# RuanJohn/Mava

Measured on AMD Instinct MI355X. Metric: env-steps/sec (whole node), ff_mappo RWARE tiny-4ag, higher is better.
Workload: dtype f32 via 2 x f16 split operands on the MFMA (3 products, f32 accumulate); 1 GPU; ff_mappo RWARE tiny-4ag-shaped synthetic obs, 4096 envs/GPU (update_batch_size=1 x num_envs=4096), rollout_length=128, ppo_epochs=4, num_minibatches=2, agents=4, obs=70/264, actions=5, one step = one PPO update = 524288 env-steps per GPU; parallelism=dp1

## Files before the change

### include/mava_hip.h

```cpp
#ifndef MAVA_HIP_H
#define MAVA_HIP_H

#include <stddef.h>
#include <stdint.h>

#ifdef __cplusplus
extern "C" {
#endif

typedef struct ihipStream_t* mava_stream_t;

const char* mava_last_error(void);
int mava_abi_version(void);

typedef struct mava_ctx mava_ctx;
enum {
  MAVA_CTX_MATMUL_MODE = 0,
  MAVA_CTX_CRITIC_AGGREGATION = 1,
  MAVA_CTX_GAE_VARIANT = 2,
  MAVA_CTX_POLICY_VARIANT = 3,
  MAVA_CTX_H2_LAUNCHES = 4,
  MAVA_CTX_TRAIN_VARIANT = 5,
  MAVA_CTX_W8_LAUNCHES = 6,
  MAVA_CTX_W1_SPLIT_FRESH = 7,
  MAVA_CTX_EXACT_TILES = 8
};
int mava_ctx_create(mava_ctx** out);
int mava_ctx_destroy(mava_ctx* ctx);
int mava_ctx_set(mava_ctx* ctx, int key, long value);
int mava_ctx_get(const mava_ctx* ctx, int key, long* value);

int mava_gae_f32(const mava_ctx* ctx, const float* reward, const float* value, const uint8_t* done,
                 const float* last_val, const uint8_t* last_done, int T, int N, float gamma,
                 float lambda, float* adv, float* tgt, mava_stream_t s);

int mava_permutation_i32(long n, uint64_t seed, uint64_t counter, int32_t* out, mava_stream_t s);

int mava_clip_adam(float* p, const float* g, float* m, float* v, int32_t* count,
                   const int* seg_off, const float* seg_lr, int n_seg, float grad_scale,
                   float max_norm, int decay, int steps_per_update, int num_updates, float b1,
// ... 363 lines not shown
```

### mava_amd/_lib.py

```python
from __future__ import annotations

import ctypes as C
import os
from typing import Optional

import torch

_HERE = os.path.dirname(os.path.abspath(__file__))
LIB_PATH = os.environ.get("MAVA_LIB_PATH") or os.path.join(_HERE, "libmavahip.so")

_lib: Optional[C.CDLL] = None


class MavaHipError(RuntimeError):
    pass


vp = C.c_void_p
i32 = C.c_int
u32 = C.c_uint32
u64 = C.c_uint64
f32 = C.c_float
lng = C.c_long

# ... 111 lines not shown
            )
        _lib = C.CDLL(LIB_PATH)
        _lib.mava_last_error.restype = C.c_char_p
        _lib.mava_last_error.argtypes = []
        for name, args in _SIGNATURES.items():
            fn = getattr(_lib, name)
            fn.argtypes = args
            fn.restype = _RESTYPES.get(name, C.c_int)
    return _lib


class Ctx:

    MATMUL_MODE, CRITIC_AGGREGATION, GAE_VARIANT, POLICY_VARIANT, H2_LAUNCHES, TRAIN_VARIANT, W8_LAUNCHES, W1_SPLIT_FRESH = 0, 1, 2, 3, 4, 5, 6, 7
    EXACT_TILES = 8

    def __init__(self, matmul_mode: str = "f32", critic_aggregation: bool = True):
        if matmul_mode not in ("f32", "f16x2"):
            raise ValueError(f"matmul_mode must be 'f16x2' or 'f32', got {matmul_mode!r}")
        h = C.c_void_p()
        check(lib().mava_ctx_create(C.byref(h)), "mava_ctx_create")
        self.handle: Optional[int] = h.value
        self.set(self.MATMUL_MODE, 1 if matmul_mode == "f16x2" else 0)
        self.set(self.CRITIC_AGGREGATION, int(bool(critic_aggregation)))

    def set(self, key: int, value: int) -> None:
        check(lib().mava_ctx_set(self.handle, key, int(value)), "mava_ctx_set")

    def get(self, key: int) -> int:
        out = C.c_long()
# ... 59 lines not shown
```

### mava_amd/csrc/api.cpp

```cpp
#include <stdarg.h>
#include <stdio.h>
#include <string.h>

#include "common.h"
#include "ctx.h"

static thread_local char g_err[512] = "";

void mava_set_error(const char* fmt, ...) {
  va_list ap;
  va_start(ap, fmt);
  vsnprintf(g_err, sizeof(g_err), fmt, ap);
  va_end(ap);
}

extern "C" const char* mava_last_error(void) { return g_err; }

extern "C" int mava_abi_version(void) { return 3; }

enum { CTX_MATMUL_MODE = 0, CTX_CRITIC_AGGREGATION = 1, CTX_GAE_VARIANT = 2, CTX_POLICY_VARIANT = 3, CTX_H2_LAUNCHES = 4, CTX_TRAIN_VARIANT = 5, CTX_W8_LAUNCHES = 6, CTX_W1_SPLIT_FRESH = 7, CTX_EXACT_TILES = 8 };

extern "C" int mava_ctx_create(mava_ctx** out) {
  MAVA_ARG_CHECK(out != nullptr, 0, "mava_ctx_create: null output pointer");
  mava_ctx* c = new mava_ctx();
  c->matmul_mode = 0;
  c->critic_aggregation = 1;
  c->gae_variant = 0;
  c->policy_variant = 0;
  c->h2_launches = 0;
  c->train_variant = 0;
  c->w8_launches = 0;
  c->w1_split[0] = c->w1_split[1] = nullptr;
  for (int i = 0; i < 2; ++i) {
    c->w1_fresh[i] = 0;
    c->w1_key_params[i] = nullptr;
    c->w1_key_din[i] = c->w1_key_steps[i] = 0;
  }
  c->exact_tiles = nullptr;
  *out = c;
  return MAVA_OK;
}

extern "C" int mava_ctx_destroy(mava_ctx* c) {
  if (c == nullptr) return MAVA_OK;
  for (int i = 0; i < 2; ++i)
    if (c->w1_split[i] != nullptr) (void)hipFree(c->w1_split[i]);
  if (c->exact_tiles != nullptr) (void)hipFree(c->exact_tiles);
  delete c;
  return MAVA_OK;
}

extern "C" int mava_ctx_set(mava_ctx* c, int key, long value) {
  MAVA_ARG_CHECK(c != nullptr, 0, "mava_ctx_set: null context");
  switch (key) {
    case CTX_MATMUL_MODE:
      MAVA_ARG_CHECK(value == 0 || value == 1, 1, "mava_ctx_set: matmul mode %ld (0 = exact f32, 1 = f16x2)", value);
      c->matmul_mode = (int)value;
      c->w1_fresh[0] = c->w1_fresh[1] = 0;
      return MAVA_OK;
    case CTX_CRITIC_AGGREGATION: c->critic_aggregation = value ? 1 : 0; return MAVA_OK;
    case CTX_GAE_VARIANT: c->gae_variant = (int)value; return MAVA_OK;
    case CTX_POLICY_VARIANT: c->policy_variant = (int)value; return MAVA_OK;
    case CTX_H2_LAUNCHES: c->h2_launches = value; return MAVA_OK;
    case CTX_TRAIN_VARIANT: c->train_variant = (int)value; return MAVA_OK;
    case CTX_W8_LAUNCHES: c->w8_launches = value; return MAVA_OK;
    case CTX_W1_SPLIT_FRESH:
      MAVA_ARG_CHECK(value == 0, 1, "mava_ctx_set: MAVA_CTX_W1_SPLIT_FRESH can only be cleared (0) by the caller");
      c->w1_fresh[0] = c->w1_fresh[1] = 0;
      return MAVA_OK;
    case CTX_EXACT_TILES:
      MAVA_ARG_CHECK(value == 0, 1, "mava_ctx_set: MAVA_CTX_EXACT_TILES can only be reset (0) by the caller");
      if (c->exact_tiles != nullptr) {
        MAVA_HIP_CHECK(hipDeviceSynchronize());
        MAVA_HIP_CHECK(hipMemset(c->exact_tiles, 0, sizeof(unsigned long long)));
      }
      return MAVA_OK;
    default: mava_set_error("mava_ctx_set: unknown key %d", key); return MAVA_EARG(2);
  }
}

extern "C" int mava_ctx_get(const mava_ctx* c, int key, long* value) {
  MAVA_ARG_CHECK(c != nullptr && value != nullptr, 0, "mava_ctx_get: null argument");
  switch (key) {
    case CTX_MATMUL_MODE: *value = c->matmul_mode; return MAVA_OK;
    case CTX_CRITIC_AGGREGATION: *value = c->critic_aggregation; return MAVA_OK;
    case CTX_GAE_VARIANT: *value = c->gae_variant; return MAVA_OK;
    case CTX_POLICY_VARIANT: *value = c->policy_variant; return MAVA_OK;
    case CTX_H2_LAUNCHES: *value = c->h2_launches; return MAVA_OK;
    case CTX_TRAIN_VARIANT: *value = c->train_variant; return MAVA_OK;
    case CTX_W8_LAUNCHES: *value = c->w8_launches; return MAVA_OK;
    case CTX_W1_SPLIT_FRESH: *value = c->w1_fresh[1]; return MAVA_OK;
    case CTX_EXACT_TILES: {
      unsigned long long n = 0;
      if (c->exact_tiles != nullptr) {
        MAVA_HIP_CHECK(hipDeviceSynchronize());
        MAVA_HIP_CHECK(hipMemcpy(&n, c->exact_tiles, sizeof(n), hipMemcpyDeviceToHost));
      }
      *value = (long)n;
      return MAVA_OK;
    }
    default: mava_set_error("mava_ctx_get: unknown key %d", key); return MAVA_EARG(2);
  }
}
```

### mava_amd/csrc/ctx.h

```cpp
#pragma once
#include "common.h"

struct mava_ctx {
  int matmul_mode;
  int critic_aggregation;
  int gae_variant;
  int policy_variant;
  int train_variant;
  long h2_launches;
  long w8_launches;
  void* w1_split[2];
  int w1_fresh[2];
  const float* w1_key_params[2];
  int w1_key_din[2];
  int w1_key_steps[2];
  unsigned long long* exact_tiles;
};

static inline int mava_ctx_matmul_mode(const mava_ctx* c) { return c ? c->matmul_mode : 0; }
static inline int mava_ctx_critic_aggregation(const mava_ctx* c) { return c ? c->critic_aggregation : 1; }
static inline int mava_ctx_gae_variant(const mava_ctx* c) { return c ? c->gae_variant : 0; }
static inline int mava_ctx_policy_variant(const mava_ctx* c) { return c ? c->policy_variant : 0; }
```

### mava_amd/csrc/ppo_train_h2.hip

```cpp
#include "h2_core.h"
#include "ppo_train_task.h"
#include "ctx.h"

#include <type_traits>

#ifndef MAVA_GW_DEPTH
#define MAVA_GW_DEPTH 0
#endif
#define GW_DEPTH MAVA_GW_DEPTH
#ifndef MAVA_GW_DEPTH_WIDE
#define MAVA_GW_DEPTH_WIDE 0
#endif

namespace {

using namespace h2;

constexpr int STATS_BLOCKS = 128;

#ifdef MAVA_STAMPS
#define STAMP_DECL unsigned long long st_prev = __builtin_readcyclecounter(), st_acc[16] = {0, 0, 0, 0, 0, 0, 0, 0, 0, 0, 0, 0, 0, 0, 0, 0};
#define STAMP(i)                                                    \
  do {                                                              \
    __builtin_amdgcn_sched_barrier(0);                              \
// ... 1010 lines not shown
    if (tk.action_f != nullptr) return 1;
    if (tk.no <= 8) return dispatch_s1<8, true>(ctx, tk, n_slab, s);
#ifndef MAVA_FAST_BUILD
    if (tk.no <= 16) return dispatch_s1<16, true>(ctx, tk, n_slab, s);
    return dispatch_s1<32, true>(ctx, tk, n_slab, s);
#else
    return 1;
#endif
  }
  return dispatch_s1<1, false>(ctx, tk, n_slab, s);
}

int mava_train_h2_launch(mava_ctx* ctx, const TrainTask& tk_in, int n_slab, bool actor, hipStream_t s) {
  TrainTask tk = tk_in;
  tk.force_xlo = (ctx->train_variant & 2) != 0;
  if ((ctx->train_variant & 1) == 0) {
    const int rc8 = mava_train_w8_launch(tk, n_slab, actor, s);
    if (rc8 <= 0) {
      if (rc8 == 0) { ++ctx->h2_launches; ++ctx->w8_launches; }
      return rc8;
    }
  }
  const int rc = h2_dispatch(ctx, tk, n_slab, actor, s);
  if (rc == 0) ++ctx->h2_launches;
  return rc;
}
```

### mava_amd/csrc/ppo_train_task.h

```cpp
#pragma once
#include <stdint.h>

#include "common.h"

struct TrainTask {
  const float* params;
  const float* x;
  int din, no, xshare, xv;
  int A;
  int agg;
  const int32_t* idx;
  long idx_base;
  int Rb;
  const uint8_t* mask;
  const int32_t* action;
  const float* action_f;
  uint32_t seed_lo, seed_hi, ent_step, row_offset;
  float min_scale;
  const float* old_logp;
  const float* adv;
  const double* stats;
  const float* old_value;
  const float* targets;
  float clip_eps, ent_coef, vf_coef;
  float* slab;
  long slab_stride;
  unsigned long long* stamps;
  int force_xlo;
  unsigned long long* exact_tiles;
};

struct mava_ctx;
int mava_train_w8_launch(const TrainTask& tk, int n_slab, bool actor, hipStream_t s);
int mava_train_h2_launch(mava_ctx* ctx, const TrainTask& tk, int n_slab, bool actor, hipStream_t s);

extern int g_train_last_instance;
constexpr int train_instance_id(int family, bool actor, bool cont, bool wide, int no, int k, int xv) {
  return family * 1000000 + ((actor ? 1 : 0) + (cont ? 2 : 0) + (wide ? 4 : 0)) * 100000 + no * 1000 + k * 10 + xv;
}
```

### mava_amd/csrc/ppo_train_w8.hip

```cpp
#include "h2_core.h"
#include "ppo_train_task.h"
#include "ctx.h"

namespace {

using namespace h2;
typedef float f32x4 __attribute__((ext_vector_type(4)));

constexpr int STATS_BLOCKS = 128;
#ifndef MAVA_W8_GWD
#define MAVA_W8_GWD 1
#endif
constexpr int GWD = MAVA_W8_GWD;

#ifdef MAVA_STAMPS
#define WSTAMP_DECL unsigned long long ws_prev = __builtin_readcyclecounter(), ws_acc[16] = {0, 0, 0, 0, 0, 0, 0, 0, 0, 0, 0, 0, 0, 0, 0, 0};
#define WSTAMP(i)                                                   \
  do {                                                              \
    __builtin_amdgcn_sched_barrier(0);                              \
    const unsigned long long ws_now = __builtin_readcyclecounter(); \
    ws_acc[i] += ws_now - ws_prev;                                  \
    ws_prev = ws_now;                                               \
    __builtin_amdgcn_sched_barrier(0);                              \
  } while (0)
#else
#define WSTAMP_DECL
#define WSTAMP(i)
#endif

struct Frag4 {
  half4 hi, lo;
};
__device__ __forceinline__ f32x4 mfma3w(const Frag& a, const Frag& b, f32x4 c) {
  c = __builtin_amdgcn_mfma_f32_16x16x32_f16(a.lo, b.hi, c, 0, 0, 0);
  c = __builtin_amdgcn_mfma_f32_16x16x32_f16(a.hi, b.lo, c, 0, 0, 0);
  return __builtin_amdgcn_mfma_f32_16x16x32_f16(a.hi, b.hi, c, 0, 0, 0);
}
__device__ __forceinline__ f32x4 mfma2w_blo0(const Frag& a, const half8& bhi, f32x4 c) {
  c = __builtin_amdgcn_mfma_f32_16x16x32_f16(a.lo, bhi, c, 0, 0, 0);
  return __builtin_amdgcn_mfma_f32_16x16x32_f16(a.hi, bhi, c, 0, 0, 0);
}
__device__ __forceinline__ f32x4 mfma2w_alo0(const half8& ahi, const Frag& b, f32x4 c) {
  c = __builtin_amdgcn_mfma_f32_16x16x32_f16(ahi, b.lo, c, 0, 0, 0);
  return __builtin_amdgcn_mfma_f32_16x16x32_f16(ahi, b.hi, c, 0, 0, 0);
// ... 27 lines not shown
struct W8Layout {
  int h1, dz2, dz1, w2, xs, dy, small, end;
};
inline W8Layout make_w8_layout() {
  W8Layout L;
  L.h1 = 0;
  L.dz2 = L.h1 + WIMG;
  L.dz1 = L.dz2 + WIMG;
  L.w2 = L.dz1 + WIMG;
  L.xs = L.w2 + 2 * W2PLANE;
  L.dy = L.xs + 2 * WIMG;
  L.small = L.dy + 2 * DYPLANE;
  L.end = L.small + (32 + 16 + 16) * 4;
  return L;
}

template <int NO, int S1, int XV, int W2R, bool ACTOR, int ROLE>
__device__ __forceinline__ void w8_body(const TrainTask& tk, const W8Layout& L, u8* lds) {
  constexpr bool DO_LOSS = ROLE != 2, DO_STAGE = ROLE != 1;
  constexpr float WS = ACTOR ? 1.0f : W_SCALE_CRITIC, WU = 1.0f / WS;
  constexpr int KT1 = 2 * S1;
  u8* const H1I = lds + L.h1;
  u8* const DZ2I = lds + L.dz2;
  u8* const DZ1I = lds + L.dz1;
  u8* const W2I = lds + L.w2;
  u8* const DYI = lds + L.dy;
  float* const YP = reinterpret_cast<float*>(lds + L.dz2);
  constexpr int YSTR = (NO == 8) ? 9 : NO;
  float* const B3s = reinterpret_cast<float*>(lds + L.small);
  float* const misc = B3s + 32;
// ... 104 lines not shown
  auto cursor_advance = [&](Cursor& c) {
    c.q += q_step; c.b += b_step; c.a += a_step;
    if (c.a >= Au) { c.a -= Au; c.b += 1u; }
  };
  auto cursor_gather = [&](const Cursor& c, int32_t& p_raw, uint32_t& a_out) {
    const bool in = c.q < (uint32_t)R;
    const uint32_t b = in ? c.b : b_last;
    a_out = in ? c.a : a_last;
    p_raw = tk.idx ? tk.idx[b] : (int32_t)(tk.idx_base + (long)b);
  };
  auto stage_row = [&](int32_t p_raw, uint32_t a) -> uint32_t {
    const uint32_t fr = (uint32_t)p_raw * Au + a;
    if constexpr (ACTOR) return fr;
    else return (tk.xshare == 1) ? fr : ((uint32_t)tk.xshare == Au ? (uint32_t)p_raw : fr / (uint32_t)tk.xshare);
  };
  auto stage_issue = [&](uint32_t fr, float (&xr)[NR]) {
    const float* xrow = tk.x + (long)fr * din;
#pragma unroll
    for (int k = 0; k < NPC; ++k) {
      const int c = l16 + TPR * k;
      const int cc = (c < nv) ? c : 0;
      if (XV == 2) {
        const float2 t = reinterpret_cast<const float2*>(xrow)[cc];
        xr[2 * k] = t.x; xr[2 * k + 1] = t.y;
      } else {
        xr[k] = xrow[cc];
      }
    }
  };
  u8* const xs_dummy = reinterpret_cast<u8*>(misc + 8);
  const int xsw = 16 * w8_sw(srow);
  auto stage_commit = [&](int buf, const float (&xr)[NR]) {
    u8* base = lds + L.xs + buf * WIMG + WROW * srow;
    uint32_t lo_any = 0;
#pragma unroll
    for (int k = 0; k < NPC; ++k) {
      const int c = l16 + TPR * k;
      const bool ok = c < nv;
      const int col = XV * c;
      u8* qa = ok ? (base + ((16 * (col >> 3)) ^ xsw) + 2 * (col & 7)) : xs_dummy;
      u8* qb = ok ? (qa + WPLANE32) : xs_dummy;
      if (XV == 2) {
        typedef _Float16 half2v __attribute__((ext_vector_type(2)));
        half2v a, b;
#pragma unroll
        for (int e = 0; e < 2; ++e) { _Float16 x0, x1; split1(xr[2 * k + e], x0, x1); a[e] = x0; b[e] = x1; }
        *reinterpret_cast<half2v*>(qa) = a;
        *reinterpret_cast<half2v*>(qb) = b;
        lo_any |= __builtin_bit_cast(uint32_t, b) & 0x7FFF7FFFu;
      } else {
        _Float16 x0, x1;
        split1(xr[k], x0, x1);
        *reinterpret_cast<_Float16*>(qa) = x0;
        *reinterpret_cast<_Float16*>(qb) = x1;
        lo_any |= (uint32_t)__builtin_bit_cast(uint16_t, x1) & 0x7FFFu;
      }
    }
    if (lo_any != 0) xflag[buf] = 1u;
  };
  auto load_row = [&](uint32_t fr, int& act, float& f0, float& f1, uint32_t& m) {
    if constexpr (ACTOR) {
      act = tk.action[fr];
      f0 = tk.old_logp[fr];
      f1 = tk.adv[fr];
      const uint8_t* mk = (tk.mask != nullptr && lo < no) ? (tk.mask + (long)fr * no + lo) : nullptr;
      m = 1u;
      if (mk != nullptr) m = *mk;
    } else {
      act = 0;
      f0 = tk.old_value[fr];
      f1 = tk.targets[fr];
      m = 0u;
    }
  };

// ... 42 lines not shown
    trA[t] = trb + ((32 * t) ^ thx);
    asm volatile("" : "+v"(trA[t]));
  }
  auto tr_addr = [&](int t) -> int { return trA[t]; };
  const int trOwn = tr_addr(v);
  auto read_tr = [&](const u8* img, int plane, int a0) -> Frag {
    Frag f;
    f.hi = read_tr8(img + a0, WROW);
    f.lo = read_tr8(img + plane + a0, WROW);
    return f;
  };
  auto read_row = [&](const u8* img, int plane, int a0) -> Frag { return read_row_frag(img, plane, a0); };
  const int dyRd = DYROW * i + 8 * kg;
  const int dyTr = DYROW * trow + 8 * tp;
  int buf = 0;

  WSTAMP_DECL
  for (; it < ntiles; it += gridDim.x, buf ^= 1) {
    WSTAMP(14);
    const long itn = it + gridDim.x;
    const bool have_next = itn < ntiles;
    const u8* const XSI = lds + L.xs + buf * WIMG;
    uint32_t xrow_next = DO_STAGE ? stage_row(ps_next, as_next) : 0u, lrow_next = DO_LOSS ? ((uint32_t)pl_next * Au + al_next) : 0u;
    if constexpr (DO_STAGE) asm volatile("" : "+v"(xrow_next));
    if constexpr (DO_LOSS) asm volatile("" : "+v"(lrow_next));

    f32x4 acc[2] = {f32x4{0, 0, 0, 0}, f32x4{0, 0, 0, 0}};
    const bool x_lo = __builtin_amdgcn_readfirstlane((int)xflag[buf]) != 0 || tk.force_xlo != 0;
    if (x_lo) {
      Frag xb[2];
#pragma unroll
      for (int nt = 0; nt < 2; ++nt) xb[nt] = read_row(XSI + 4096 * nt, WPLANE32, rdA[0]);
#pragma unroll
      for (int s = 0; s < S1; ++s) {
        Frag b[2] = {xb[0], xb[1]};
        if (s + 1 < S1) {
#pragma unroll
          for (int nt = 0; nt < 2; ++nt) xb[nt] = read_row(XSI + 4096 * nt, WPLANE32, rdA[(s + 1) & 3]);
        }
#pragma unroll
        for (int nt = 0; nt < 2; ++nt) acc[nt] = mfma3w(W1f[s], b[nt], acc[nt]);
        __builtin_amdgcn_sched_barrier(0);
      }
    } else {
      half8 xb[2];
#pragma unroll
      for (int nt = 0; nt < 2; ++nt) xb[nt] = *reinterpret_cast<const half8*>(XSI + 4096 * nt + rdA[0]);
#pragma unroll
      for (int s = 0; s < S1; ++s) {
        const half8 b[2] = {xb[0], xb[1]};
        if (s + 1 < S1) {
#pragma unroll
          for (int nt = 0; nt < 2; ++nt) xb[nt] = *reinterpret_cast<const half8*>(XSI + 4096 * nt + rdA[(s + 1) & 3]);
        }
#pragma unroll
        for (int nt = 0; nt < 2; ++nt) acc[nt] = mfma2w_blo0(W1f[s], b[nt], acc[nt]);
        __builtin_amdgcn_sched_barrier(0);
      }
    }
    WSTAMP(0);
    uint32_t relu1 = 0;
#pragma unroll
    for (int nt = 0; nt < 2; ++nt) {
#pragma unroll
      for (int r = 0; r < 4; ++r) {
        acc[nt][r] = fmaxf(ACTOR ? acc[nt][r] : acc[nt][r] * WU, 0.0f);
        relu1 |= (acc[nt][r] > 0.0f) ? (1u << (4 * nt + r)) : 0u;
      }
      const Frag4 f = split4(acc[nt]);
      *reinterpret_cast<half4*>(H1I + 4096 * nt + wrA) = f.hi;
      *reinterpret_cast<half4*>(H1I + 4096 * nt + WPLANE32 + wrA) = f.lo;
    }
    WSTAMP(1);
    if (have_next) {
      if constexpr (DO_STAGE) stage_issue(xrow_next, xr);
      if constexpr (DO_LOSS) load_row(lrow_next, n_act, n_f0, n_f1, n_m);
      if (itn + gridDim.x < ntiles) {
        if constexpr (DO_STAGE) { cursor_gather(cs, ps_next, as_next); cursor_advance(cs); }
        if constexpr (DO_LOSS) { cursor_gather(cl, pl_next, al_next); cursor_advance(cl); }
      }
    }
    WSTAMP(2);
    __syncthreads();
    WSTAMP(3);
    if constexpr (DO_STAGE) {
      if (tid == (ROLE == 2 ? 256 : 0)) xflag[buf ^ 1] = 0u;
    }

    f32x4 h2[2];
#pragma unroll
    for (int nt = 0; nt < 2; ++nt) h2[nt] = f32x4{b2r[0], b2r[1], b2r[2], b2r[3]};
    {
      Frag hb[2], wn;
#pragma unroll
      for (int nt = 0; nt < 2; ++nt) hb[nt] = read_row(H1I + 4096 * nt, WPLANE32, rdA[0]);
      if constexpr (W2R < 1) wn = read_tr(W2I, W2PLANE, trOwn);
#pragma unroll
      for (int s = 0; s < 4; ++s) {
        Frag b[2] = {hb[0], hb[1]};
        const Frag a = (s < W2R) ? W2f[s < W2R ? s : 0] : wn;
        if (s + 1 < 4) {
#pragma unroll
          for (int nt = 0; nt < 2; ++nt) hb[nt] = read_row(H1I + 4096 * nt, WPLANE32, rdA[s + 1]);
          if (s + 1 >= W2R) wn = read_tr(W2I + 32 * (s + 1) * WROW, W2PLANE, trOwn);
        }
#pragma unroll
        for (int nt = 0; nt < 2; ++nt) h2[nt] = mfma3w(a, b[nt], h2[nt]);
        __builtin_amdgcn_sched_barrier(0);
      }
    }
    WSTAMP(4);
    uint32_t relu2 = 0;
#pragma unroll
    for (int nt = 0; nt < 2; ++nt) {
#pragma unroll
      for (int r = 0; r < 4; ++r) {
        h2[nt][r] = fmaxf(ACTOR ? h2[nt][r] : h2[nt][r] * WU, 0.0f);
        relu2 |= (h2[nt][r] > 0.0f) ? (1u << (4 * nt + r)) : 0u;
      }
      const Frag4 f = split4(h2[nt]);
      *reinterpret_cast<half4*>(DZ1I + 4096 * nt + wrA) = f.hi;
      *reinterpret_cast<half4*>(DZ1I + 4096 * nt + WPLANE32 + wrA) = f.lo;
      const f32x4 y = mfma3k16(W3h, f, f32x4{0, 0, 0, 0});
#pragma unroll
      for (int r = 0; r < 4; ++r) {
        if (4 * kg + r < NO) YP[(v * 32 + 16 * nt + i) * YSTR + 4 * kg + r] = y[r] * W3_UNSCALE;
      }
    }
    WSTAMP(5);
    __syncthreads();
    WSTAMP(6);

    if constexpr (DO_LOSS) {
      const float lo_c = 1.0f - tk.clip_eps, hi_c = 1.0f + tk.clip_eps;
      const bool rvalid = (it * 32 + lrow) < R;
      const float* yp = YP + lrow * YSTR + lo;
      float y = B3s[lo];
#pragma unroll
      for (int u = 0; u < 8; ++u) y += yp[u * 32 * YSTR];
      float dyo = 0.0f, pg_row = 0.0f, ent_row = 0.0f;
      if constexpr (ACTOR) {
        const bool legal = (lo < no) && (r_m != 0u);
        const float z = legal ? y : -FLT_MAX;
        auto fmax_op = [](float a, float b) { return fmaxf(a, b); };
        auto add_op = [](float a, float b) { return a + b; };
        const float mx = group_allreduce<NO>(z, fmax_op);
        const float se = group_allreduce<NO>(expf(z - mx), add_op);
        const float logp = (mx == -FLT_MAX) ? ((lo < no) ? -logf((float)no) : -FLT_MAX) : z - (mx + logf(se));
        const float pr = expf(logp);
        const float ent = group_allreduce<NO>((pr > 0.0f) ? -(pr * logp) : 0.0f, add_op);
        const int act = r_act;
        const float lp = group_allreduce<NO>((lo == act) ? logp : 0.0f, add_op);
        const float gae = (r_f1 - adv_mean) * adv_rstd;
        const float ratio = expf(lp - r_f0);
        const float rc = fminf(fmaxf(ratio, lo_c), hi_c);
        const float l1 = ratio * gae, l2 = rc * gae;
        const float pg = -fminf(l1, l2);
        const bool inside = (ratio >= lo_c) && (ratio <= hi_c);
        const float g1 = (l1 < l2) ? 1.0f : ((l1 == l2) ? 0.5f : 0.0f);
        const float g2 = inside ? (1.0f - g1) : 0.0f;
        const float dlp = rvalid ? (-(g1 + g2) * gae * ratio) : 0.0f;
        const float ec = rvalid ? tk.ent_coef : 0.0f;
        const float oh = (lo == act) ? 1.0f : 0.0f;
        const float pl2 = (pr > 0.0f) ? logp : 0.0f;
        dyo = dlp * (oh - pr) + ec * pr * (pl2 + ent);
        if (z == -FLT_MAX) dyo = 0.0f;
        pg_row = pg;
// ... 10 lines not shown
        dyo = (rvalid && lo == 0) ? (tk.vf_coef * (g1 * e1 + g2 * e2)) : 0.0f;
        pg_row = 0.5f * fmaxf(l1, l2);
      }
      _Float16 da, db;
      split1(dyo, da, db);
      *reinterpret_cast<_Float16*>(DYI + lrow * DYROW + 2 * lo) = da;
      *reinterpret_cast<_Float16*>(DYI + DYPLANE + lrow * DYROW + 2 * lo) = db;
      ab3 += dyo;
      if (rvalid && lo == 0) {
        loss_a += pg_row * invR;
        loss_b += ent_row * invR;
      }
      r_act = n_act; r_f0 = n_f0; r_f1 = n_f1; r_m = n_m;
    }
    if constexpr (DO_STAGE) {
      if (have_next) stage_commit(buf ^ 1, xr);
    }
    WSTAMP(7);
    __syncthreads();
    WSTAMP(8);

    {
      Frag a, b;
      a.hi = read_tr8(DYI + dyTr, DYROW);
      a.lo = read_tr8(DYI + DYPLANE + dyTr, DYROW);
      b = read_tr(DZ1I, WPLANE32, trOwn);
      gW3 = mfma3w(a, b, gW3);
    }
    f32x4 dz[2];
#pragma unroll
    for (int nt = 0; nt < 2; ++nt) {
      Frag4 b;
      b.hi = *reinterpret_cast<const half4*>(DYI + 16 * nt * DYROW + dyRd);
      b.lo = *reinterpret_cast<const half4*>(DYI + DYPLANE + 16 * nt * DYROW + dyRd);
      dz[nt] = mfma3k16(W3d, b, f32x4{0, 0, 0, 0});
#pragma unroll
      for (int r = 0; r < 4; ++r) {
        dz[nt][r] = ((relu2 >> (4 * nt + r)) & 1u) ? dz[nt][r] * W3_UNSCALE : 0.0f;
        ab2[r] += dz[nt][r];
      }
      const Frag4 f = split4(dz[nt]);
      *reinterpret_cast<half4*>(DZ2I + 4096 * nt + wrA) = f.hi;
      *reinterpret_cast<half4*>(DZ2I + 4096 * nt + WPLANE32 + wrA) = f.lo;
    }
    WSTAMP(9);
    {
      const Frag b = read_tr(DZ2I, WPLANE32, trOwn);
      Frag an[GWD];
#pragma unroll
      for (int t = 0; t < GWD; ++t) an[t] = read_tr(H1I, WPLANE32, tr_addr(t));
#pragma unroll
      for (int t = 0; t < 8; ++t) {
        const Frag a = an[t % GWD];
        if (t + GWD < 8) an[t % GWD] = read_tr(H1I, WPLANE32, tr_addr(t + GWD));
        gW2[t] = mfma3w(a, b, gW2[t]);
        __builtin_amdgcn_sched_barrier(0);
      }
    }
    WSTAMP(10);
    __syncthreads();
    WSTAMP(11);

    {
      acc[0] = f32x4{0, 0, 0, 0};
      acc[1] = f32x4{0, 0, 0, 0};
      Frag an = read_row(W2I + 4096 * v, W2PLANE, rdA[0]);
      Frag bn[2];
#pragma unroll
      for (int nt = 0; nt < 2; ++nt) bn[nt] = read_row(DZ2I + 4096 * nt, WPLANE32, rdA[0]);
#pragma unroll
      for (int s = 0; s < 4; ++s) {
        const Frag a = an;
        Frag b[2] = {bn[0], bn[1]};
        if (s + 1 < 4) {
          an = read_row(W2I + 4096 * v, W2PLANE, rdA[s + 1]);
#pragma unroll
          for (int nt = 0; nt < 2; ++nt) bn[nt] = read_row(DZ2I + 4096 * nt, WPLANE32, rdA[s + 1]);
        }
#pragma unroll
        for (int nt = 0; nt < 2; ++nt) acc[nt] = mfma3w(a, b[nt], acc[nt]);
        __builtin_amdgcn_sched_barrier(0);
      }
#pragma unroll
      for (int nt = 0; nt < 2; ++nt) {
#pragma unroll
        for (int r = 0; r < 4; ++r) acc[nt][r] = ((relu1 >> (4 * nt + r)) & 1u) ? (ACTOR ? acc[nt][r] : acc[nt][r] * WU) : 0.0f;
        const Frag4 f = split4(acc[nt]);
        *reinterpret_cast<half4*>(DZ1I + 4096 * nt + wrA) = f.hi;
        *reinterpret_cast<half4*>(DZ1I + 4096 * nt + WPLANE32 + wrA) = f.lo;
      }
    }
    WSTAMP(12);
    {
      const Frag b = read_tr(DZ1I, WPLANE32, trOwn);
      constexpr int D1 = GWD < KT1 ? GWD : KT1;
      if (x_lo) {
        Frag an[D1];
#pragma unroll
        for (int t = 0; t < D1; ++t) an[t] = read_tr(XSI, WPLANE32, tr_addr(t));
#pragma unroll
        for (int t = 0; t < KT1; ++t) {
          const Frag a = an[t % D1];
          if (t + D1 < KT1) an[t % D1] = read_tr(XSI, WPLANE32, tr_addr(t + D1));
          gW1[t] = mfma3w(a, b, gW1[t]);
          __builtin_amdgcn_sched_barrier(0);
        }
      } else {
        half8 an[D1];
#pragma unroll
        for (int t = 0; t < D1; ++t) an[t] = read_tr8(XSI + tr_addr(t), WROW);
#pragma unroll
        for (int t = 0; t < KT1; ++t) {
          const half8 a = an[t % D1];
          if (t + D1 < KT1) an[t % D1] = read_tr8(XSI + tr_addr(t + D1), WROW);
          gW1[t] = mfma2w_alo0(a, b, gW1[t]);
          __builtin_amdgcn_sched_barrier(0);
        }
      }
    }
    WSTAMP(13);
  }
#ifdef MAVA_STAMPS
  if (tk.stamps != nullptr && blockIdx.x == 0 && l == 0) {
    for (int k = 0; k < 16; ++k) tk.stamps[v * 16 + k] = ws_acc[k];
  }
#endif

  __syncthreads();
  float* slab = tk.slab + (long)blockIdx.x * tk.slab_stride;
  const int oB2 = mlp_off_b2(din), oB3 = mlp_off_b3(din, no);
  const int Pn = mlp_param_count(din, no);
#pragma unroll
  for (int t = 0; t < KT1; ++t)
#pragma unroll
    for (int r = 0; r < 4; ++r) {
      const int k = 16 * t + 4 * kg + r;
      if (k <= din) slab[k * MLP_H + 16 * v + i] = gW1[t][r] * invR;
    }
#pragma unroll
  for (int t = 0; t < 8; ++t)
#pragma unroll
    for (int r = 0; r < 4; ++r) slab[oW2 + (16 * t + 4 * kg + r) * MLP_H + 16 * v + i] = gW2[t][r] * invR;
#pragma unroll
  for (int r = 0; r < 4; ++r) {
    float x = ab2[r];
#pragma unroll
    for (int m = 1; m < 16; m <<= 1) x += __shfl_xor(x, m, 64);
    if (i == 0) slab[oB2 + 16 * v + 4 * kg + r] = x * invR;
    const int o = 4 * kg + r;
    if (o < no) slab[oW3 + (16 * v + i) * no + o] = gW3[r] * invR;
  }
  float* red = reinterpret_cast<float*>(lds + L.h1);
  if constexpr (DO_LOSS) {
    float x = ab3;
#pragma unroll
    for (int m = NO; m < 64; m <<= 1) x += __shfl_xor(x, m, 64);
    if (l < NO) red[v * NO + l] = x;
    for (int o = 32; o > 0; o >>= 1) {
      loss_a += __shfl_down(loss_a, o, 64);
      loss_b += __shfl_down(loss_b, o, 64);
    }
    if (l == 0) { red[8 * NO + 2 * v] = loss_a; red[8 * NO + 2 * v + 1] = loss_b; }
  }
  __syncthreads();
  constexpr int LW = LOSS_THREADS / 64;
  if (tid < no) {
    float x = 0.0f;
#pragma unroll
    for (int u = 0; u < LW; ++u) x += red[u * NO + tid];
    slab[oB3 + tid] = x * invR;
  }
  if (tid == 0) {
    float a = 0.0f, b = 0.0f;
#pragma unroll
    for (int u = 0; u < LW; ++u) { a += red[8 * NO + 2 * u]; b += red[8 * NO + 2 * u + 1]; }
    slab[Pn] = a;
    slab[Pn + 1] = b;
  }
}

constexpr int w8_w2r(int no, int s1, int xv) {
#ifdef MAVA_W8_W2R
  return MAVA_W8_W2R;
#else
  return (no == 8) ? ((s1 <= 2) ? 2 : ((s1 == 3 && xv == 2) ? 2 : 0)) : ((s1 <= 2) ? 2 : 0);
#endif
}
// ... 65 lines not shown
```

Baseline: 78.30 million env-steps/s.

## Add triple-buffered ring in w8 train kernel overlapping next-tile layer-1 MFMAs

Adds a three-slot ring of x staging buffers to the fused w8 PPO training kernel for NO==8 and S1<=3 configs. While the input tiles' f16 low parts stay zero, it skips storing the low plane and computes the next tile's layer-1 forward MFMAs early, interleaved with the actor loss softmax reductions or after the layer-2 sync. When a nonzero low part shows up it drains back to the original two-buffer exact path. This hides layer-1 latency behind the loss math and cuts LDS writes, at the cost of more registers, a bigger code path, and a new counter plus a ctx key for diagnostics.

New measurement: 78.53 million env-steps/s (median of 6 runs). About the same (+0.3%).

```diff
diff --git a/include/mava_hip.h b/include/mava_hip.h
--- a/include/mava_hip.h
+++ b/include/mava_hip.h
@@ -23,7 +23,8 @@
   MAVA_CTX_TRAIN_VARIANT = 5,
   MAVA_CTX_W8_LAUNCHES = 6,
   MAVA_CTX_W1_SPLIT_FRESH = 7,
-  MAVA_CTX_EXACT_TILES = 8
+  MAVA_CTX_EXACT_TILES = 8,
+  MAVA_CTX_W8_EXACT_TILES = 9
 };
 int mava_ctx_create(mava_ctx** out);
 int mava_ctx_destroy(mava_ctx* ctx);
diff --git a/mava_amd/_lib.py b/mava_amd/_lib.py
--- a/mava_amd/_lib.py
+++ b/mava_amd/_lib.py
@@ -149,6 +149,7 @@
 
     MATMUL_MODE, CRITIC_AGGREGATION, GAE_VARIANT, POLICY_VARIANT, H2_LAUNCHES, TRAIN_VARIANT, W8_LAUNCHES, W1_SPLIT_FRESH = 0, 1, 2, 3, 4, 5, 6, 7
     EXACT_TILES = 8
+    W8_EXACT_TILES = 9
 
     def __init__(self, matmul_mode: str = "f32", critic_aggregation: bool = True):
         if matmul_mode not in ("f32", "f16x2"):
diff --git a/mava_amd/csrc/api.cpp b/mava_amd/csrc/api.cpp
--- a/mava_amd/csrc/api.cpp
+++ b/mava_amd/csrc/api.cpp
@@ -18,7 +18,7 @@
 
 extern "C" int mava_abi_version(void) { return 3; }
 
-enum { CTX_MATMUL_MODE = 0, CTX_CRITIC_AGGREGATION = 1, CTX_GAE_VARIANT = 2, CTX_POLICY_VARIANT = 3, CTX_H2_LAUNCHES = 4, CTX_TRAIN_VARIANT = 5, CTX_W8_LAUNCHES = 6, CTX_W1_SPLIT_FRESH = 7, CTX_EXACT_TILES = 8 };
+enum { CTX_MATMUL_MODE = 0, CTX_CRITIC_AGGREGATION = 1, CTX_GAE_VARIANT = 2, CTX_POLICY_VARIANT = 3, CTX_H2_LAUNCHES = 4, CTX_TRAIN_VARIANT = 5, CTX_W8_LAUNCHES = 6, CTX_W1_SPLIT_FRESH = 7, CTX_EXACT_TILES = 8, CTX_W8_EXACT_TILES = 9 };
 
 extern "C" int mava_ctx_create(mava_ctx** out) {
   MAVA_ARG_CHECK(out != nullptr, 0, "mava_ctx_create: null output pointer");
@@ -37,6 +37,7 @@
     c->w1_key_din[i] = c->w1_key_steps[i] = 0;
   }
   c->exact_tiles = nullptr;
+  c->w8_exact_tiles = nullptr;
   *out = c;
   return MAVA_OK;
 }
@@ -46,6 +47,7 @@
   for (int i = 0; i < 2; ++i)
     if (c->w1_split[i] != nullptr) (void)hipFree(c->w1_split[i]);
   if (c->exact_tiles != nullptr) (void)hipFree(c->exact_tiles);
+  if (c->w8_exact_tiles != nullptr) (void)hipFree(c->w8_exact_tiles);
   delete c;
   return MAVA_OK;
 }
@@ -69,12 +71,15 @@
       c->w1_fresh[0] = c->w1_fresh[1] = 0;
       return MAVA_OK;
     case CTX_EXACT_TILES:
-      MAVA_ARG_CHECK(value == 0, 1, "mava_ctx_set: MAVA_CTX_EXACT_TILES can only be reset (0) by the caller");
-      if (c->exact_tiles != nullptr) {
+    case CTX_W8_EXACT_TILES: {
+      MAVA_ARG_CHECK(value == 0, 1, "mava_ctx_set: the exact-tile counters can only be reset (0) by the caller");
+      unsigned long long* const word = (key == CTX_EXACT_TILES) ? c->exact_tiles : c->w8_exact_tiles;
+      if (word != nullptr) {
         MAVA_HIP_CHECK(hipDeviceSynchronize());
-        MAVA_HIP_CHECK(hipMemset(c->exact_tiles, 0, sizeof(unsigned long long)));
+        MAVA_HIP_CHECK(hipMemset(word, 0, sizeof(unsigned long long)));
       }
       return MAVA_OK;
+    }
     default: mava_set_error("mava_ctx_set: unknown key %d", key); return MAVA_EARG(2);
   }
 }
@@ -90,11 +95,13 @@
     case CTX_TRAIN_VARIANT: *value = c->train_variant; return MAVA_OK;
     case CTX_W8_LAUNCHES: *value = c->w8_launches; return MAVA_OK;
     case CTX_W1_SPLIT_FRESH: *value = c->w1_fresh[1]; return MAVA_OK;
-    case CTX_EXACT_TILES: {
+    case CTX_EXACT_TILES:
+    case CTX_W8_EXACT_TILES: {
       unsigned long long n = 0;
-      if (c->exact_tiles != nullptr) {
+      const unsigned long long* const word = (key == CTX_EXACT_TILES) ? c->exact_tiles : c->w8_exact_tiles;
+      if (word != nullptr) {
         MAVA_HIP_CHECK(hipDeviceSynchronize());
-        MAVA_HIP_CHECK(hipMemcpy(&n, c->exact_tiles, sizeof(n), hipMemcpyDeviceToHost));
+        MAVA_HIP_CHECK(hipMemcpy(&n, word, sizeof(n), hipMemcpyDeviceToHost));
       }
       *value = (long)n;
       return MAVA_OK;
diff --git a/mava_amd/csrc/ctx.h b/mava_amd/csrc/ctx.h
--- a/mava_amd/csrc/ctx.h
+++ b/mava_amd/csrc/ctx.h
@@ -15,6 +15,7 @@
   int w1_key_din[2];
   int w1_key_steps[2];
   unsigned long long* exact_tiles;
+  unsigned long long* w8_exact_tiles;
 };
 
 static inline int mava_ctx_matmul_mode(const mava_ctx* c) { return c ? c->matmul_mode : 0; }
diff --git a/mava_amd/csrc/ppo_train_h2.hip b/mava_amd/csrc/ppo_train_h2.hip
--- a/mava_amd/csrc/ppo_train_h2.hip
+++ b/mava_amd/csrc/ppo_train_h2.hip
@@ -1048,7 +1048,15 @@
 int mava_train_h2_launch(mava_ctx* ctx, const TrainTask& tk_in, int n_slab, bool actor, hipStream_t s) {
   TrainTask tk = tk_in;
   tk.force_xlo = (ctx->train_variant & 2) != 0;
+  tk.w8_no_ring = (ctx->train_variant & 4) != 0;
   if ((ctx->train_variant & 1) == 0) {
+    if (ctx->w8_exact_tiles == nullptr) {
+      void* word = nullptr;
+      MAVA_HIP_CHECK(hipMalloc(&word, sizeof(unsigned long long)));
+      ctx->w8_exact_tiles = static_cast<unsigned long long*>(word);
+      MAVA_HIP_CHECK(hipMemsetAsync(word, 0, sizeof(unsigned long long), s));
+    }
+    tk.w8_exact_tiles = ctx->w8_exact_tiles;
     const int rc8 = mava_train_w8_launch(tk, n_slab, actor, s);
     if (rc8 <= 0) {
       if (rc8 == 0) { ++ctx->h2_launches; ++ctx->w8_launches; }
diff --git a/mava_amd/csrc/ppo_train_task.h b/mava_amd/csrc/ppo_train_task.h
--- a/mava_amd/csrc/ppo_train_task.h
+++ b/mava_amd/csrc/ppo_train_task.h
@@ -27,7 +27,9 @@
   long slab_stride;
   unsigned long long* stamps;
   int force_xlo;
+  int w8_no_ring;
   unsigned long long* exact_tiles;
+  unsigned long long* w8_exact_tiles;
 };
 
 struct mava_ctx;
diff --git a/mava_amd/csrc/ppo_train_w8.hip b/mava_amd/csrc/ppo_train_w8.hip
--- a/mava_amd/csrc/ppo_train_w8.hip
+++ b/mava_amd/csrc/ppo_train_w8.hip
@@ -14,7 +14,10 @@
 constexpr int GWD = MAVA_W8_GWD;
 
 #ifdef MAVA_STAMPS
-#define WSTAMP_DECL unsigned long long ws_prev = __builtin_readcyclecounter(), ws_acc[16] = {0, 0, 0, 0, 0, 0, 0, 0, 0, 0, 0, 0, 0, 0, 0, 0};
+#define WSTAMP_DECL                                          \
+  unsigned long long ws_prev = __builtin_readcyclecounter(); \
+  unsigned long long ws_acc[32];                             \
+  for (int ws_k = 0; ws_k < 32; ++ws_k) ws_acc[ws_k] = 0;
 #define WSTAMP(i)                                                   \
   do {                                                              \
     __builtin_amdgcn_sched_barrier(0);                              \
@@ -28,6 +31,14 @@
 #define WSTAMP(i)
 #endif
 
+template <bool B>
+struct BoolTag {
+  static constexpr bool value = B;
+};
+template <int N>
+struct IntTag {
+  static constexpr int value = N;
+};
 struct Frag4 {
   half4 hi, lo;
 };
@@ -85,6 +96,8 @@
   L.end = L.small + (32 + 16 + 16) * 4;
   return L;
 }
+
+constexpr bool w8_ring(int no, int s1) { return no == 8 && s1 <= 3; }
 
 template <int NO, int S1, int XV, int W2R, bool ACTOR, int ROLE>
 __device__ __forceinline__ void w8_body(const TrainTask& tk, const W8Layout& L, u8* lds) {
@@ -219,7 +232,7 @@
     if constexpr (ACTOR) return fr;
     else return (tk.xshare == 1) ? fr : ((uint32_t)tk.xshare == Au ? (uint32_t)p_raw : fr / (uint32_t)tk.xshare);
   };
-  auto stage_issue = [&](uint32_t fr, float (&xr)[NR]) {
+  auto stage_issue = [&](uint32_t fr, float (&xr)[NR]) __attribute__((always_inline)) {
     const float* xrow = tk.x + (long)fr * din;
 #pragma unroll
     for (int k = 0; k < NPC; ++k) {
@@ -235,8 +248,10 @@
   };
   u8* const xs_dummy = reinterpret_cast<u8*>(misc + 8);
   const int xsw = 16 * w8_sw(srow);
-  auto stage_commit = [&](int buf, const float (&xr)[NR]) {
-    u8* base = lds + L.xs + buf * WIMG + WROW * srow;
+  unsigned* const ring_flag = reinterpret_cast<unsigned*>(misc + 4);
+  auto commit_rows = [&](auto lo_tag, int xoff, unsigned* flag, const float (&xr)[NR]) __attribute__((always_inline)) {
+    constexpr bool LO = decltype(lo_tag)::value;
+    u8* base = lds + L.xs + xoff + WROW * srow;
     uint32_t lo_any = 0;
 #pragma unroll
     for (int k = 0; k < NPC; ++k) {
@@ -251,19 +266,21 @@
 #pragma unroll
         for (int e = 0; e < 2; ++e) { _Float16 x0, x1; split1(xr[2 * k + e], x0, x1); a[e] = x0; b[e] = x1; }
         *reinterpret_cast<half2v*>(qa) = a;
-        *reinterpret_cast<half2v*>(qb) = b;
+        if constexpr (LO) *reinterpret_cast<half2v*>(qb) = b;
         lo_any |= __builtin_bit_cast(uint32_t, b) & 0x7FFF7FFFu;
       } else {
         _Float16 x0, x1;
         split1(xr[k], x0, x1);
         *reinterpret_cast<_Float16*>(qa) = x0;
-        *reinterpret_cast<_Float16*>(qb) = x1;
+        if constexpr (LO) *reinterpret_cast<_Float16*>(qb) = x1;
         lo_any |= (uint32_t)__builtin_bit_cast(uint16_t, x1) & 0x7FFFu;
       }
     }
-    if (lo_any != 0) xflag[buf] = 1u;
-  };
-  auto load_row = [&](uint32_t fr, int& act, float& f0, float& f1, uint32_t& m) {
+    if (lo_any != 0) *flag = 1u;
+  };
+  auto stage_commit = [&](int buf, const float (&xr)[NR]) __attribute__((always_inline)) { commit_rows(BoolTag<true>{}, buf * WIMG, xflag + buf, xr); };
+  auto stage_commit_hi = [&](int xoff, const float (&xr)[NR]) __attribute__((always_inline)) { commit_rows(BoolTag<false>{}, xoff, ring_flag, xr); };
+  auto load_row = [&](uint32_t fr, int& act, float& f0, float& f1, uint32_t& m) __attribute__((always_inline)) {
     if constexpr (ACTOR) {
       act = tk.action[fr];
       f0 = tk.old_logp[fr];
@@ -336,51 +353,67 @@
   const int dyRd = DYROW * i + 8 * kg;
   const int dyTr = DYROW * trow + 8 * tp;
   int buf = 0;
-
+  auto layer1_hi = [&](const u8* X, f32x4 (&z)[2], auto fence_tag) __attribute__((always_inline)) {
+    z[0] = f32x4{0, 0, 0, 0};
+    z[1] = f32x4{0, 0, 0, 0};
+    half8 xb[2];
+#pragma unroll
+    for (int nt = 0; nt < 2; ++nt) xb[nt] = *reinterpret_cast<const half8*>(X + 4096 * nt + rdA[0]);
+#pragma unroll
+    for (int s = 0; s < S1; ++s) {
+      const half8 b[2] = {xb[0], xb[1]};
+      if (s + 1 < S1) {
+#pragma unroll
+        for (int nt = 0; nt < 2; ++nt) xb[nt] = *reinterpret_cast<const half8*>(X + 4096 * nt + rdA[(s + 1) & 3]);
+      }
+#pragma unroll
+      for (int nt = 0; nt < 2; ++nt) z[nt] = mfma2w_blo0(W1f[s], b[nt], z[nt]);
+      if constexpr (decltype(fence_tag)::value) __builtin_amdgcn_sched_barrier(0);
+    }
+  };
+
+  f32x4 acc[2], accn[2];
+  int xo0 = 0, xo1 = WPLANE32, xo2 = 2 * WPLANE32;
+  bool leave = false;
   WSTAMP_DECL
-  for (; it < ntiles; it += gridDim.x, buf ^= 1) {
-    WSTAMP(14);
+  auto tile = [&](auto ex_tag) __attribute__((always_inline)) {
+    constexpr bool EX = decltype(ex_tag)::value;
+    constexpr int SB = EX ? 16 : 0;
+    WSTAMP(SB + 14);
     const long itn = it + gridDim.x;
-    const bool have_next = itn < ntiles;
-    const u8* const XSI = lds + L.xs + buf * WIMG;
+    const bool have_next = itn < ntiles, have_next2 = itn + gridDim.x < ntiles;
+    const bool drain = EX && leave;
+    const int bufL = (xo0 == 2 * WPLANE32) ? 0 : 1;
+    const u8* const XSI = lds + L.xs + (EX ? xo0 : buf * WIMG);
     uint32_t xrow_next = DO_STAGE ? stage_row(ps_next, as_next) : 0u, lrow_next = DO_LOSS ? ((uint32_t)pl_next * Au + al_next) : 0u;
     if constexpr (DO_STAGE) asm volatile("" : "+v"(xrow_next));
     if constexpr (DO_LOSS) asm volatile("" : "+v"(lrow_next));
 
-    f32x4 acc[2] = {f32x4{0, 0, 0, 0}, f32x4{0, 0, 0, 0}};
-    const bool x_lo = __builtin_amdgcn_readfirstlane((int)xflag[buf]) != 0 || tk.force_xlo != 0;
-    if (x_lo) {
-      Frag xb[2];
-#pragma unroll
-      for (int nt = 0; nt < 2; ++nt) xb[nt] = read_row(XSI + 4096 * nt, WPLANE32, rdA[0]);
-#pragma unroll
-      for (int s = 0; s < S1; ++s) {
-        Frag b[2] = {xb[0], xb[1]};
-        if (s + 1 < S1) {
-#pragma unroll
-          for (int nt = 0; nt < 2; ++nt) xb[nt] = read_row(XSI + 4096 * nt, WPLANE32, rdA[(s + 1) & 3]);
+    bool x_lo = false;
+    if constexpr (!EX) {
+      x_lo = __builtin_amdgcn_readfirstlane((int)xflag[buf]) != 0 || tk.force_xlo != 0;
+      if (x_lo) {
+        acc[0] = f32x4{0, 0, 0, 0};
+        acc[1] = f32x4{0, 0, 0, 0};
+        Frag xb[2];
+#pragma unroll
+        for (int nt = 0; nt < 2; ++nt) xb[nt] = read_row(XSI + 4096 * nt, WPLANE32, rdA[0]);
+#pragma unroll
+        for (int s = 0; s < S1; ++s) {
+          Frag b[2] = {xb[0], xb[1]};
+          if (s + 1 < S1) {
+#pragma unroll
+            for (int nt = 0; nt < 2; ++nt) xb[nt] = read_row(XSI + 4096 * nt, WPLANE32, rdA[(s + 1) & 3]);
+          }
+#pragma unroll
+          for (int nt = 0; nt < 2; ++nt) acc[nt] = mfma3w(W1f[s], b[nt], acc[nt]);
+          __builtin_amdgcn_sched_barrier(0);
         }
-#pragma unroll
-        for (int nt = 0; nt < 2; ++nt) acc[nt] = mfma3w(W1f[s], b[nt], acc[nt]);
-        __builtin_amdgcn_sched_barrier(0);
-      }
-    } else {
-      half8 xb[2];
-#pragma unroll
-      for (int nt = 0; nt < 2; ++nt) xb[nt] = *reinterpret_cast<const half8*>(XSI + 4096 * nt + rdA[0]);
-#pragma unroll
-      for (int s = 0; s < S1; ++s) {
-        const half8 b[2] = {xb[0], xb[1]};
-        if (s + 1 < S1) {
-#pragma unroll
-          for (int nt = 0; nt < 2; ++nt) xb[nt] = *reinterpret_cast<const half8*>(XSI + 4096 * nt + rdA[(s + 1) & 3]);
-        }
-#pragma unroll
-        for (int nt = 0; nt < 2; ++nt) acc[nt] = mfma2w_blo0(W1f[s], b[nt], acc[nt]);
-        __builtin_amdgcn_sched_barrier(0);
-      }
-    }
-    WSTAMP(0);
+      } else {
+        layer1_hi(XSI, acc, BoolTag<true>{});
+      }
+    }
+    WSTAMP(SB + 0);
     uint32_t relu1 = 0;
 #pragma unroll
     for (int nt = 0; nt < 2; ++nt) {
@@ -393,19 +426,32 @@
       *reinterpret_cast<half4*>(H1I + 4096 * nt + wrA) = f.hi;
       *reinterpret_cast<half4*>(H1I + 4096 * nt + WPLANE32 + wrA) = f.lo;
     }
-    WSTAMP(1);
-    if (have_next) {
+    WSTAMP(SB + 1);
+    if constexpr (EX) {
+      if constexpr (DO_STAGE) {
+        if (!drain && have_next2) {
+          stage_issue(xrow_next, xr);
+          if (itn + 2 * (long)gridDim.x < ntiles) { cursor_gather(cs, ps_next, as_next); cursor_advance(cs); }
+        }
+      }
+      if constexpr (DO_LOSS) {
+        if (have_next) {
+          load_row(lrow_next, n_act, n_f0, n_f1, n_m);
+          if (have_next2) { cursor_gather(cl, pl_next, al_next); cursor_advance(cl); }
+        }
+      }
+    } else if (have_next) {
       if constexpr (DO_STAGE) stage_issue(xrow_next, xr);
       if constexpr (DO_LOSS) load_row(lrow_next, n_act, n_f0, n_f1, n_m);
-      if (itn + gridDim.x < ntiles) {
+      if (have_next2) {
         if constexpr (DO_STAGE) { cursor_gather(cs, ps_next, as_next); cursor_advance(cs); }
         if constexpr (DO_LOSS) { cursor_gather(cl, pl_next, al_next); cursor_advance(cl); }
       }
     }
-    WSTAMP(2);
+    WSTAMP(SB + 2);
     __syncthreads();
-    WSTAMP(3);
-    if constexpr (DO_STAGE) {
+    WSTAMP(SB + 3);
+    if constexpr (DO_STAGE && !EX) {
       if (tid == (ROLE == 2 ? 256 : 0)) xflag[buf ^ 1] = 0u;
     }
 
@@ -431,7 +477,7 @@
         __builtin_amdgcn_sched_barrier(0);
       }
     }
-    WSTAMP(4);
+    WSTAMP(SB + 4);
     uint32_t relu2 = 0;
 #pragma unroll
     for (int nt = 0; nt < 2; ++nt) {
@@ -449,10 +495,37 @@
         if (4 * kg + r < NO) YP[(v * 32 + 16 * nt + i) * YSTR + 4 * kg + r] = y[r] * W3_UNSCALE;
       }
     }
-    WSTAMP(5);
+    WSTAMP(SB + 5);
     __syncthreads();
-    WSTAMP(6);
-
+    WSTAMP(SB + 6);
+
+    if constexpr (EX) {
+      accn[0] = f32x4{0, 0, 0, 0};
+      accn[1] = f32x4{0, 0, 0, 0};
+    }
+    half8 xe[2][2];
+    auto early_reads = [&](auto s_tag) __attribute__((always_inline)) {
+      constexpr int s = decltype(s_tag)::value;
+      if constexpr (EX && s < S1) {
+#pragma unroll
+        for (int nt = 0; nt < 2; ++nt) xe[s & 1][nt] = *reinterpret_cast<const half8*>(lds + L.xs + xo1 + 4096 * nt + rdA[s & 3]);
+      }
+    };
+    auto early_group = [&](auto g_tag) __attribute__((always_inline)) {
+      constexpr int g = decltype(g_tag)::value, s = g / 2;
+      if constexpr (EX && g < 2 * S1) {
+        if constexpr (g % 2 == 0) early_reads(IntTag<s + 1>{});
+#pragma unroll
+        for (int nt = 0; nt < 2; ++nt)
+          accn[nt] = __builtin_amdgcn_mfma_f32_16x16x32_f16(g % 2 == 0 ? W1f[s].lo : W1f[s].hi, xe[s & 1][nt], accn[nt], 0, 0, 0);
+        __builtin_amdgcn_sched_barrier(0);
+      }
+    };
+    early_reads(IntTag<0>{});
+    if constexpr (!(DO_LOSS && ACTOR)) {
+      early_group(IntTag<0>{}); early_group(IntTag<1>{}); early_group(IntTag<2>{});
+      early_group(IntTag<3>{}); early_group(IntTag<4>{}); early_group(IntTag<5>{});
+    }
     if constexpr (DO_LOSS) {
       const float lo_c = 1.0f - tk.clip_eps, hi_c = 1.0f + tk.clip_eps;
       const bool rvalid = (it * 32 + lrow) < R;
@@ -462,17 +535,23 @@
       for (int u = 0; u < 8; ++u) y += yp[u * 32 * YSTR];
       float dyo = 0.0f, pg_row = 0.0f, ent_row = 0.0f;
       if constexpr (ACTOR) {
+        early_group(IntTag<0>{});
         const bool legal = (lo < no) && (r_m != 0u);
         const float z = legal ? y : -FLT_MAX;
         auto fmax_op = [](float a, float b) { return fmaxf(a, b); };
         auto add_op = [](float a, float b) { return a + b; };
         const float mx = group_allreduce<NO>(z, fmax_op);
+        early_group(IntTag<1>{});
         const float se = group_allreduce<NO>(expf(z - mx), add_op);
+        early_group(IntTag<2>{});
         const float logp = (mx == -FLT_MAX) ? ((lo < no) ? -logf((float)no) : -FLT_MAX) : z - (mx + logf(se));
         const float pr = expf(logp);
+        early_group(IntTag<3>{});
         const float ent = group_allreduce<NO>((pr > 0.0f) ? -(pr * logp) : 0.0f, add_op);
+        early_group(IntTag<4>{});
         const int act = r_act;
         const float lp = group_allreduce<NO>((lo == act) ? logp : 0.0f, add_op);
+        early_group(IntTag<5>{});
         const float gae = (r_f1 - adv_mean) * adv_rstd;
         const float ratio = expf(lp - r_f0);
         const float rc = fminf(fmaxf(ratio, lo_c), hi_c);
@@ -513,11 +592,19 @@
       r_act = n_act; r_f0 = n_f0; r_f1 = n_f1; r_m = n_m;
     }
     if constexpr (DO_STAGE) {
-      if (have_next) stage_commit(buf ^ 1, xr);
-    }
-    WSTAMP(7);
+      if constexpr (EX) {
+        if (drain) stage_commit(bufL, xr);
+        else if (have_next2) stage_commit_hi(xo2, xr);
+      } else {
+        if (have_next) stage_commit(buf ^ 1, xr);
+      }
+    }
+    WSTAMP(SB + 7);
     __syncthreads();
-    WSTAMP(8);
+    WSTAMP(SB + 8);
+    if constexpr (EX) {
+      if (!drain) leave = __builtin_amdgcn_readfirstlane((int)*ring_flag) != 0;
+    }
 
     {
       Frag a, b;
@@ -542,7 +629,7 @@
       *reinterpret_cast<half4*>(DZ2I + 4096 * nt + wrA) = f.hi;
       *reinterpret_cast<half4*>(DZ2I + 4096 * nt + WPLANE32 + wrA) = f.lo;
     }
-    WSTAMP(9);
+    WSTAMP(SB + 9);
     {
       const Frag b = read_tr(DZ2I, WPLANE32, trOwn);
       Frag an[GWD];
@@ -556,9 +643,9 @@
         __builtin_amdgcn_sched_barrier(0);
       }
     }
-    WSTAMP(10);
+    WSTAMP(SB + 10);
     __syncthreads();
-    WSTAMP(11);
+    WSTAMP(SB + 11);
 
     {
       acc[0] = f32x4{0, 0, 0, 0};
@@ -589,7 +676,7 @@
         *reinterpret_cast<half4*>(DZ1I + 4096 * nt + WPLANE32 + wrA) = f.lo;
       }
     }
-    WSTAMP(12);
+    WSTAMP(SB + 12);
     {
       const Frag b = read_tr(DZ1I, WPLANE32, trOwn);
       constexpr int D1 = GWD < KT1 ? GWD : KT1;
@@ -617,15 +704,69 @@
         }
       }
     }
-    WSTAMP(13);
-  }
+    WSTAMP(SB + 13);
+  };
+
+  long n_ring = 0;
+  constexpr bool RING = w8_ring(NO, S1);
+  if constexpr (RING) {
+    if (it < ntiles && tk.w8_no_ring == 0 && tk.force_xlo == 0 && __builtin_amdgcn_readfirstlane((int)xflag[0]) == 0) {
+      if (tid < 32) *reinterpret_cast<_Float16*>(lds + L.xs + WPLANE32 + w8_off(tid, din >> 3) + 2 * (din & 7)) = (_Float16)1.0f;
+      const bool have_next = it + gridDim.x < ntiles;
+      if constexpr (DO_STAGE) {
+        if (have_next) {
+          stage_issue(stage_row(ps_next, as_next), xr);
+          if (it + 2 * (long)gridDim.x < ntiles) { cursor_gather(cs, ps_next, as_next); cursor_advance(cs); }
+        }
+      }
+      layer1_hi(lds + L.xs, acc, BoolTag<true>{});
+      if constexpr (DO_STAGE) {
+        if (have_next) stage_commit_hi(xo1, xr);
+      }
+      __syncthreads();
+      leave = __builtin_amdgcn_readfirstlane((int)*ring_flag) != 0;
+      bool left = false;
+      while (it < ntiles) {
+        const bool drain = leave;
+        tile(BoolTag<true>{});
+        ++n_ring;
+        it += gridDim.x;
+        if (drain) {
+          buf = (xo0 == 2 * WPLANE32) ? 0 : 1;
+          left = true;
+          break;
+        }
+        acc[0] = accn[0];
+        acc[1] = accn[1];
+        const int xo = xo0;
+        xo0 = xo1;
+        xo1 = xo2;
+        xo2 = xo;
+      }
+      if (left) {
+        __syncthreads();
+        if (tid < 32) *reinterpret_cast<_Float16*>(lds + L.xs + WPLANE32 + w8_off(tid, din >> 3) + 2 * (din & 7)) = (_Float16)0.0f;
+        __syncthreads();
+      }
+    }
+  }
+  for (; it < ntiles; it += gridDim.x, buf ^= 1) tile(BoolTag<false>{});
 #ifdef MAVA_STAMPS
   if (tk.stamps != nullptr && blockIdx.x == 0 && l == 0) {
-    for (int k = 0; k < 16; ++k) tk.stamps[v * 16 + k] = ws_acc[k];
+    for (int k = 0; k < 16; ++k) {
+      tk.stamps[v * 16 + k] = ws_acc[k];
+      tk.stamps[128 + v * 16 + k] = ws_acc[16 + k];
+    }
   }
 #endif
+  if constexpr (RING) {
+    if (tid == 0 && tk.w8_exact_tiles != nullptr && n_ring > 0) atomicAdd(tk.w8_exact_tiles, (unsigned long long)n_ring);
+  }
 
   __syncthreads();
+  int tid_e = tid;
+  asm volatile("" : "+v"(tid_e));
+  const int l_e = tid_e & 63, v_e = tid_e >> 6, i_e = l_e & 15, kg_e = l_e >> 4;
   float* slab = tk.slab + (long)blockIdx.x * tk.slab_stride;
   const int oB2 = mlp_off_b2(din), oB3 = mlp_off_b3(din, no);
   const int Pn = mlp_param_count(din, no);
@@ -633,43 +774,43 @@
   for (int t = 0; t < KT1; ++t)
 #pragma unroll
     for (int r = 0; r < 4; ++r) {
-      const int k = 16 * t + 4 * kg + r;
-      if (k <= din) slab[k * MLP_H + 16 * v + i] = gW1[t][r] * invR;
+      const int k = 16 * t + 4 * kg_e + r;
+      if (k <= din) slab[k * MLP_H + 16 * v_e + i_e] = gW1[t][r] * invR;
     }
 #pragma unroll
   for (int t = 0; t < 8; ++t)
 #pragma unroll
-    for (int r = 0; r < 4; ++r) slab[oW2 + (16 * t + 4 * kg + r) * MLP_H + 16 * v + i] = gW2[t][r] * invR;
+    for (int r = 0; r < 4; ++r) slab[oW2 + (16 * t + 4 * kg_e + r) * MLP_H + 16 * v_e + i_e] = gW2[t][r] * invR;
 #pragma unroll
   for (int r = 0; r < 4; ++r) {
     float x = ab2[r];
 #pragma unroll
     for (int m = 1; m < 16; m <<= 1) x += __shfl_xor(x, m, 64);
-    if (i == 0) slab[oB2 + 16 * v + 4 * kg + r] = x * invR;
-    const int o = 4 * kg + r;
-    if (o < no) slab[oW3 + (16 * v + i) * no + o] = gW3[r] * invR;
+    if (i_e == 0) slab[oB2 + 16 * v_e + 4 * kg_e + r] = x * invR;
+    const int o = 4 * kg_e + r;
+    if (o < no) slab[oW3 + (16 * v_e + i_e) * no + o] = gW3[r] * invR;
   }
   float* red = reinterpret_cast<float*>(lds + L.h1);
   if constexpr (DO_LOSS) {
     float x = ab3;
 #pragma unroll
     for (int m = NO; m < 64; m <<= 1) x += __shfl_xor(x, m, 64);
-    if (l < NO) red[v * NO + l] = x;
+    if (l_e < NO) red[v_e * NO + l_e] = x;
     for (int o = 32; o > 0; o >>= 1) {
       loss_a += __shfl_down(loss_a, o, 64);
       loss_b += __shfl_down(loss_b, o, 64);
     }
-    if (l == 0) { red[8 * NO + 2 * v] = loss_a; red[8 * NO + 2 * v + 1] = loss_b; }
+    if (l_e == 0) { red[8 * NO + 2 * v_e] = loss_a; red[8 * NO + 2 * v_e + 1] = loss_b; }
   }
   __syncthreads();
   constexpr int LW = LOSS_THREADS / 64;
-  if (tid < no) {
+  if (tid_e < no) {
     float x = 0.0f;
 #pragma unroll
-    for (int u = 0; u < LW; ++u) x += red[u * NO + tid];
-    slab[oB3 + tid] = x * invR;
-  }
-  if (tid == 0) {
+    for (int u = 0; u < LW; ++u) x += red[u * NO + tid_e];
+    slab[oB3 + tid_e] = x * invR;
+  }
+  if (tid_e == 0) {
     float a = 0.0f, b = 0.0f;
 #pragma unroll
     for (int u = 0; u < LW; ++u) { a += red[8 * NO + 2 * u]; b += red[8 * NO + 2 * u + 1]; }
```
